# zju3dv/NeuralRecon-W

Hardware: NVIDIA H100
Metric: training rays/sec (higher is better)
Workload: dtype bf16 (3-product split forward, plain bf16 backward, fp32 accumulate)

## Files before the change

### neuralrecon-w_b200/csrc/epilogue_fast.cuh

```cuda
#pragma once
#include "epilogue_tc.cuh"

namespace nrw {

enum EpiKind {
  EK_GENERIC = 0,
  EK_FWD_SOFTPLUS,
  EK_FWD_RELU,
  EK_FWD_NONE,
  EK_GATE_FWD,
  EK_TANGENT,
  EK_REVERSE,
  EK_RELU_BWD,
  EK_FWD_HEAD,
  EK_COUNT
};

inline int pick_epi_kind(const Epi& e) {
  auto al16 = [](const void* p) { return (reinterpret_cast<uintptr_t>(p) & 15) == 0; };
  auto rows16 = [&](const void* p, int ld) { return !p || (al16(p) && (ld & 3) == 0); };
  if (e.head_w || e.head_partial)
    return (e.head_w && e.head_partial && e.bias && al16(e.bias) && al16(e.head_w) && e.act == ACT_SOFTPLUS100 && e.scale == 1.0f && e.n_planes == 0 &&
            !e.atomic && !e.aux_u.p && !e.rowvec && !e.aux_relu && !e.out_pre && !e.out2 && !e.out_f32 &&
            !e.colsum && !e.aux_add && e.n_store >= (1 << 29)) ? EK_FWD_HEAD : -1;
  if (e.atomic || e.n_planes > 3) return EK_GENERIC;
  if (e.n_planes > 0 && (!al16(e.out_pl.p) || (e.out_pl.ld & 3) || (e.out_pl.pstride & 7))) return EK_GENERIC;
  if (e.aux_u.p && (!al16(e.aux_u.p) || (e.aux_u.ld & 3) || (e.aux_u.pstride & 7))) return EK_GENERIC;
  if (!rows16(e.out_pre.p, e.out_pre.ld) || !rows16(e.out2.p, e.out2.ld) || !rows16(e.aux_add.p, e.aux_add.ld) ||
      !rows16(e.aux_q.p, e.aux_q_bcast ? 0 : e.aux_q.ld) || !rows16(e.out_f32, e.ld_f32) || !rows16(e.aux_relu, e.ld_relu) ||
      !al16(e.bias) || !al16(e.colvec))
    return EK_GENERIC;
  const bool gate = e.aux_u.p != nullptr;
  if (gate && e.out_pre && !e.out2 && !e.aux_add && !e.colsum && !e.bias && !e.rowvec && !e.aux_relu && e.n_planes > 0 && !e.out_f32)
    return EK_GATE_FWD;
  if (gate && e.out2 && e.aux_q && !e.out_pre && !e.bias && !e.rowvec && !e.aux_add && !e.colsum && !e.aux_relu &&
      ((e.n_planes > 0) != (e.out_f32 != nullptr)))
    return EK_TANGENT;
  if (gate && e.aux_add && !e.out2 && !e.out_pre && !e.bias && !e.aux_relu && e.n_planes > 0 && !e.out_f32) return EK_REVERSE;
  if (!gate && e.aux_relu && !e.out_pre && !e.out2 && !e.aux_add && !e.bias && e.n_planes > 0 && !e.out_f32 && e.act == ACT_NONE)
    return EK_RELU_BWD;
  if (!gate && e.bias && !e.rowvec && !e.aux_relu && !e.aux_add && !e.out_pre && !e.out2 && !e.out_f32 && !e.colsum && e.n_planes > 0) {
    if (e.act == ACT_SOFTPLUS100) return EK_FWD_SOFTPLUS;
    if (e.act == ACT_RELU) return EK_FWD_RELU;
    if (e.act == ACT_NONE) return EK_FWD_NONE;
  }
  return EK_GENERIC;
}

#define NRW_GATE_K (-144.269504088896341f)

template <int EK>
__device__ __forceinline__ void epi_fast16(const Epi& e, float* stg, const float (&v)[16], int m0w, int nc, int M, int N, int lane,
                                           float* cs_tile, float* hacc) {
  if constexpr (EK == EK_GENERIC) {
    epi_chunk16(e, stg, v, m0w, nc, M, N, lane, cs_tile);
  } else if constexpr (EK == EK_FWD_HEAD) {
    const int col = nc + (lane & 3) * 4;
    const float4 b = ldg4(e.bias + col), hw = ldg4(e.head_w + col);
    float x[16];
    line_transpose(stg, v, lane, x);
#pragma unroll
    for (int it = 0; it < 4; ++it) {
      float p = softplus100(x[4 * it] + b.x) * hw.x;
      p = fmaf(softplus100(x[4 * it + 1] + b.y), hw.y, p);
      p = fmaf(softplus100(x[4 * it + 2] + b.z), hw.z, p);
      p = fmaf(softplus100(x[4 * it + 3] + b.w), hw.w, p);
      p += __shfl_xor_sync(0xFFFFFFFFu, p, 1);
      p += __shfl_xor_sync(0xFFFFFFFFu, p, 2);
      hacc[it] += p;
    }
  } else {
    if (M - m0w < 32 || N - nc < 16 || e.n_store - nc < 16) {
      epi_chunk16(e, stg, v, m0w, nc, M, N, lane, cs_tile);
      return;
    }
    const int col = nc + (lane & 3) * 4;
    const long long row = (long long)m0w + (lane >> 2);
    float u[16];
    float s[16];
    float4 b;
    if constexpr (EK == EK_GATE_FWD || EK == EK_TANGENT || EK == EK_REVERSE) {
      tile_load_bf16(e.aux_u.p + row * e.aux_u.ld + col, e.aux_u.ld, u);
      if constexpr (EK == EK_GATE_FWD) {
        if (e.aux_u_planes > 1) tile_load_bf16(e.aux_u.plane(1) + row * e.aux_u.ld + col, e.aux_u.ld, s);
      }
    }
    if constexpr (EK == EK_FWD_SOFTPLUS || EK == EK_FWD_RELU || EK == EK_FWD_NONE) b = ldg4(e.bias + col);
    if constexpr (EK == EK_TANGENT) {
      if (e.aux_q_bcast) {
        const float4 qb = ldg4(e.aux_q.f32() + col);
#pragma unroll
        for (int it = 0; it < 4; ++it) { s[4 * it] = qb.x; s[4 * it + 1] = qb.y; s[4 * it + 2] = qb.z; s[4 * it + 3] = qb.w; }
      } else {
        tile_load(e.aux_q, row, col, s);
      }
    }
    if constexpr (EK == EK_REVERSE) tile_load(e.aux_add, row, col, s);
    if constexpr (EK == EK_RELU_BWD) tile_load_bf16(e.aux_relu + row * e.ld_relu + col, e.ld_relu, u);
    float x[16], w[16];
    line_transpose(stg, v, lane, x);

    if constexpr (EK == EK_FWD_SOFTPLUS || EK == EK_FWD_RELU || EK == EK_FWD_NONE) {
      const float bb[4] = {b.x, b.y, b.z, b.w};
#pragma unroll
      for (int i = 0; i < 16; ++i) {
        const float t = x[i] + bb[i & 3];
        if constexpr (EK == EK_FWD_SOFTPLUS) w[i] = softplus100(t) * e.scale;
        else if constexpr (EK == EK_FWD_RELU) w[i] = fmaxf(t, 0.0f) * e.scale;
        else w[i] = t * e.scale;
      }
    }
    if constexpr (EK == EK_REVERSE || EK == EK_RELU_BWD) {
      if (e.rowvec) {
        const float4 c = ldg4(e.colvec + col);
        const float cc[4] = {c.x, c.y, c.z, c.w};
#pragma unroll
        for (int it = 0; it < 4; ++it) {
          const float rv = __ldg(e.rowvec + row + it * 8);
#pragma unroll
          for (int k = 0; k < 4; ++k) x[4 * it + k] = fmaf(rv, cc[k], x[4 * it + k]);
        }
      }
    }
    if constexpr (EK == EK_GATE_FWD) tile_store(e.out_pre, row, col, x);
    if constexpr (EK == EK_GATE_FWD || EK == EK_TANGENT || EK == EK_REVERSE) {
      if constexpr (EK == EK_GATE_FWD) {
        if (e.aux_u_planes > 1) {
#pragma unroll
          for (int i = 0; i < 16; ++i) u[i] += s[i];
        }
      }
      for (int pl = EK == EK_GATE_FWD ? 2 : 1; pl < e.aux_u_planes; ++pl) {
        float t[16];
        tile_load_bf16(e.aux_u.plane(pl) + row * e.aux_u.ld + col, e.aux_u.ld, t);
#pragma unroll
        for (int i = 0; i < 16; ++i) u[i] += t[i];
      }
      const float kk = NRW_GATE_K * e.aux_u_scale, sc = e.scale;
      if constexpr (EK == EK_TANGENT) {
        const float sc100 = 100.0f * sc;
#pragma unroll
        for (int i = 0; i < 16; ++i) {
          const float ee = mufu_ex2(u[i] * kk);
          const float s1 = 1.0f - ee;
          const float xs = x[i] * s1;
          w[i] = xs * sc;
          s[i] = (xs * s[i]) * (ee * sc100);
        }
        tile_store(e.out2, row, col, s);
      } else if constexpr (EK == EK_REVERSE) {
#pragma unroll
        for (int i = 0; i < 16; ++i) {
          const float ee = mufu_ex2(u[i] * kk);
          w[i] = fmaf(x[i], fmaf(-sc, ee, sc), s[i]);
        }
      } else {
#pragma unroll
        for (int i = 0; i < 16; ++i) {
          const float ee = mufu_ex2(u[i] * kk);
          w[i] = x[i] * fmaf(-sc, ee, sc);
        }
      }
    }
    if constexpr (EK == EK_RELU_BWD) {
#pragma unroll
      for (int i = 0; i < 16; ++i) w[i] = u[i] > 0.0f ? x[i] * e.scale : 0.0f;
    }
    if constexpr (EK == EK_REVERSE || EK == EK_RELU_BWD) {
      if (cs_tile) line_colsum_add(w, lane, cs_tile);
    }
    if constexpr (EK == EK_TANGENT) {
      if (e.out_f32) tile_store_f32(e.out_f32 + row * e.ld_f32 + col, e.ld_f32, w);
    }
    for (int pl = 0; pl < e.n_planes; ++pl) {
      uint32_t pk[8];
      if (pl + 1 < e.n_planes) split_plane<16>(w, pk);
      else pack_bf16(w, pk);
      tile_store_bf16(e.out_pl.plane(pl) + row * e.out_pl.ld + col, e.out_pl.ld, pk);
    }
  }
}

}
```

### neuralrecon-w_b200/csrc/epilogue_tc.cuh

```cuda
#pragma once
#include "epilogue.cuh"

namespace nrw {

struct LineLayout {
  int sl;
  int r0;
  int rows_valid;
  bool full;
};

__device__ __forceinline__ bool aligned16(const void* p) { return (reinterpret_cast<uintptr_t>(p) & 15) == 0; }
__device__ __forceinline__ bool aligned8(const void* p) { return (reinterpret_cast<uintptr_t>(p) & 7) == 0; }

__device__ __forceinline__ void line_transpose(float* stg, const float (&v)[16], int lane, float (&x)[16]) {
  const int sl = lane & 3, r0 = lane >> 2;
#pragma unroll
  for (int s = 0; s < 4; ++s)
    *reinterpret_cast<float4*>(stg + lane * 16 + ((s ^ ((lane >> 1) & 3)) << 2)) = make_float4(v[4 * s], v[4 * s + 1], v[4 * s + 2], v[4 * s + 3]);
  __syncwarp();
#pragma unroll
  for (int it = 0; it < 4; ++it) {
    const int rr = it * 8 + r0;
    const float4 t = *reinterpret_cast<const float4*>(stg + rr * 16 + ((sl ^ ((rr >> 1) & 3)) << 2));
    x[4 * it] = t.x; x[4 * it + 1] = t.y; x[4 * it + 2] = t.z; x[4 * it + 3] = t.w;
  }
  __syncwarp();
}

__device__ __forceinline__ float4 ldg4(const float* p) {
  float4 v;
  asm volatile("ld.global.nc.L2::256B.v4.f32 {%0, %1, %2, %3}, [%4];" : "=f"(v.x), "=f"(v.y), "=f"(v.z), "=f"(v.w) : "l"(p));
  return v;
}
__device__ __forceinline__ uint2 ldg2u(const bf16* p) {
  uint2 v;
  asm volatile("ld.global.nc.L2::256B.v2.u32 {%0, %1}, [%2];" : "=r"(v.x), "=r"(v.y) : "l"(p));
  return v;
}

__device__ __forceinline__ void tile_load_f32(const float* p, long long ld, float (&o)[16]) {
#pragma unroll
  for (int it = 0; it < 4; ++it) {
    const float4 t = ldg4(p + it * 8 * ld);
    o[4 * it] = t.x; o[4 * it + 1] = t.y; o[4 * it + 2] = t.z; o[4 * it + 3] = t.w;
  }
}
__device__ __forceinline__ void tile_load_bf16(const bf16* p, long long ld, float (&o)[16]) {
#pragma unroll
  for (int it = 0; it < 4; ++it) {
    const uint2 t = ldg2u(p + it * 8 * ld);
    o[4 * it] = __uint_as_float(t.x << 16); o[4 * it + 1] = __uint_as_float(t.x & 0xFFFF0000u);
    o[4 * it + 2] = __uint_as_float(t.y << 16); o[4 * it + 3] = __uint_as_float(t.y & 0xFFFF0000u);
  }
}
__device__ __forceinline__ void tile_store_f32(float* p, long long ld, const float (&o)[16]) {
#pragma unroll
  for (int it = 0; it < 4; ++it)
    *reinterpret_cast<float4*>(p + it * 8 * ld) = make_float4(o[4 * it], o[4 * it + 1], o[4 * it + 2], o[4 * it + 3]);
}
__device__ __forceinline__ void tile_store_bf16(bf16* p, long long ld, const uint32_t (&pk)[8]) {
#pragma unroll
  for (int it = 0; it < 4; ++it) *reinterpret_cast<uint2*>(p + it * 8 * ld) = make_uint2(pk[2 * it], pk[2 * it + 1]);
}
__device__ __forceinline__ void pack_bf16(const float (&w)[16], uint32_t (&pk)[8]) {
#pragma unroll
  for (int t = 0; t < 8; ++t) {
    const __nv_bfloat162 h = __floats2bfloat162_rn(w[2 * t], w[2 * t + 1]);
    pk[t] = *reinterpret_cast<const uint32_t*>(&h);
  }
}
__device__ __forceinline__ void tile_load(const SideStream& s, long long row, int col, float (&o)[16]) {
  if (s.is_bf16()) tile_load_bf16(s.h() + row * s.ld + col, s.ld, o);
  else tile_load_f32(s.f32() + row * s.ld + col, s.ld, o);
}
__device__ __forceinline__ void tile_store(const SideStream& s, long long row, int col, const float (&o)[16]) {
  if (s.is_bf16()) {
    uint32_t pk[8];
    pack_bf16(o, pk);
    tile_store_bf16(s.h() + row * s.ld + col, s.ld, pk);
  } else {
    tile_store_f32(s.f32() + row * s.ld + col, s.ld, o);
  }
}

__device__ __forceinline__ bool line_fast(const LineLayout& L, const void* p, long long ld, int ncols) {
  return L.full && ncols >= 16 && aligned16(p) && (ld & 3) == 0;
}
__device__ __forceinline__ void line_load_f32(const LineLayout& L, const float* __restrict__ src, long long ld, int ncols,
                                              float (&o)[16]) {
  if (line_fast(L, src, ld, ncols)) {
    tile_load_f32(src + L.r0 * ld + L.sl * 4, ld, o);
    return;
  }
#pragma unroll
  for (int it = 0; it < 4; ++it) {
    const int rr = it * 8 + L.r0;
#pragma unroll
    for (int k = 0; k < 4; ++k) {
      const int c = L.sl * 4 + k;
      o[4 * it + k] = (rr < L.rows_valid && c < ncols) ? src[(long long)rr * ld + c] : 0.0f;
    }
  }
}
__device__ __forceinline__ void line_store_f32(const LineLayout& L, float* __restrict__ dst, long long ld, int ncols,
                                               const float (&o)[16], bool atomic) {
  if (!atomic && line_fast(L, dst, ld, ncols)) {
    tile_store_f32(dst + L.r0 * ld + L.sl * 4, ld, o);
    return;
  }
#pragma unroll
  for (int it = 0; it < 4; ++it) {
    const int rr = it * 8 + L.r0;
#pragma unroll
    for (int k = 0; k < 4; ++k) {
      const int c = L.sl * 4 + k;
      if (rr < L.rows_valid && c < ncols) {
        if (atomic) atomicAdd(dst + (long long)rr * ld + c, o[4 * it + k]);
        else dst[(long long)rr * ld + c] = o[4 * it + k];
      }
    }
  }
}
__device__ __forceinline__ void line_store_bf16(const LineLayout& L, bf16* __restrict__ dst, long long ld, int ncols,
                                                const uint32_t (&pk)[8]) {
  if (L.full && ncols >= 16 && aligned8(dst) && (ld & 3) == 0) {
    tile_store_bf16(dst + L.r0 * ld + L.sl * 4, ld, pk);
    return;
  }
#pragma unroll
  for (int it = 0; it < 4; ++it) {
// ... 9 lines not shown
__device__ __forceinline__ void line_load_planes(const LineLayout& L, const Planes& P, int n_planes, long long m0w, int nc, int ncols,
                                                 float scale, float (&o)[16]) {
#pragma unroll
  for (int i = 0; i < 16; ++i) o[i] = 0.0f;
  for (int pl = 0; pl < n_planes; ++pl) {
    const bf16* src = P.plane(pl) + m0w * P.ld + nc;
    if (L.full && ncols >= 16 && aligned8(src) && (P.ld & 3) == 0) {
      float t[16];
      tile_load_bf16(src + L.r0 * P.ld + L.sl * 4, P.ld, t);
#pragma unroll
      for (int i = 0; i < 16; ++i) o[i] += t[i];
    } else {
#pragma unroll
      for (int it = 0; it < 4; ++it) {
        const int rr = it * 8 + L.r0;
#pragma unroll
        for (int k = 0; k < 4; ++k) {
          const int c = L.sl * 4 + k;
          if (rr < L.rows_valid && c < ncols) o[4 * it + k] += __bfloat162float(src[(long long)rr * P.ld + c]);
        }
      }
    }
  }
  if (scale != 1.0f) {
#pragma unroll
    for (int i = 0; i < 16; ++i) o[i] *= scale;
  }
}
__device__ __forceinline__ void line_load_cols(const LineLayout& L, const float* __restrict__ vec, int ncols, float (&b)[4]) {
  const float* p = vec + L.sl * 4;
  if (ncols >= 16 && aligned16(vec)) {
    const float4 t = __ldg(reinterpret_cast<const float4*>(p));
    b[0] = t.x; b[1] = t.y; b[2] = t.z; b[3] = t.w;
  } else {
#pragma unroll
    for (int k = 0; k < 4; ++k) b[k] = (L.sl * 4 + k < ncols) ? p[k] : 0.0f;
  }
}
__device__ __forceinline__ void line_load(const LineLayout& L, const SideStream& s, long long m0w, int nc, int ncols, float (&o)[16]) {
  if (s.is_bf16()) line_load_planes(L, Planes{s.h(), 0, s.ld}, 1, m0w, nc, ncols, 1.0f, o);
  else line_load_f32(L, s.f32() + m0w * s.ld + nc, s.ld, ncols, o);
}
__device__ __forceinline__ void line_store(const LineLayout& L, const SideStream& s, long long m0w, int nc, int ncols,
                                           const float (&o)[16]) {
  if (s.is_bf16()) {
    uint32_t pk[8];
    pack_bf16(o, pk);
    line_store_bf16(L, s.h() + m0w * s.ld + nc, s.ld, ncols, pk);
  } else {
    line_store_f32(L, s.f32() + m0w * s.ld + nc, s.ld, ncols, o, false);
  }
}

__device__ __forceinline__ void line_colsum_add(const float (&w)[16], int lane, float* cs_tile) {
  float c0 = (w[0] + w[4]) + (w[8] + w[12]), c1 = (w[1] + w[5]) + (w[9] + w[13]);
  float c2 = (w[2] + w[6]) + (w[10] + w[14]), c3 = (w[3] + w[7]) + (w[11] + w[15]);
  const bool hi16 = (lane & 16) != 0, hi8 = (lane & 8) != 0;
  const float s0 = hi16 ? c0 : c2, s1 = hi16 ? c1 : c3;
  float k0 = hi16 ? c2 : c0, k1 = hi16 ? c3 : c1;
  k0 += __shfl_xor_sync(0xFFFFFFFFu, s0, 16);
  k1 += __shfl_xor_sync(0xFFFFFFFFu, s1, 16);
  const float s = hi8 ? k0 : k1;
  float k = hi8 ? k1 : k0;
  k += __shfl_xor_sync(0xFFFFFFFFu, s, 8);
  k += __shfl_xor_sync(0xFFFFFFFFu, k, 4);
  if ((lane & 4) == 0) atomicAdd(cs_tile + (lane & 3) * 4 + (hi16 ? 2 : 0) + (hi8 ? 1 : 0), k);
}

__device__ __forceinline__ void epi_chunk16(const Epi& e, float* stg, const float (&v)[16], int m0w, int nc, int M, int N, int lane,
                                            float* cs_tile) {
  LineLayout L;
  L.rows_valid = min(32, M - m0w);
  if (L.rows_valid <= 0) return;
  const int n_all = min(N - nc, 16);
  const int n_st = min(e.n_store - nc, n_all);
  L.sl = lane & 3;
  L.r0 = lane >> 2;
  L.full = L.rows_valid == 32;
  float x[16];
  line_transpose(stg, v, lane, x);
  if (e.bias) {
    float b[4];
    line_load_cols(L, e.bias + nc, n_all, b);
#pragma unroll
    for (int i = 0; i < 16; ++i) x[i] += b[i & 3];
  }
  if (e.rowvec) {
    float cv[4];
    line_load_cols(L, e.colvec + nc, n_all, cv);
#pragma unroll
    for (int it = 0; it < 4; ++it) {
      const float rv = e.rowvec[min(m0w + it * 8 + L.r0, M - 1)];
#pragma unroll
      for (int k = 0; k < 4; ++k) x[4 * it + k] = fmaf(rv, cv[k], x[4 * it + k]);
    }
  }
  if (e.out_pre) line_store(L, e.out_pre, m0w, nc, n_all, x);
  if (n_st <= 0) return;
  if (e.atomic) {
    if (e.scale != 1.0f) {
#pragma unroll
      for (int i = 0; i < 16; ++i) x[i] *= e.scale;
    }
    line_store_f32(L, e.out_f32 + (long long)m0w * e.ld_f32 + nc, e.ld_f32, n_st, x, true);
    return;
  }
  float w[16];
  if (e.aux_u.p) {
    float a[16];
    line_load_planes(L, e.aux_u, e.aux_u_planes, m0w, nc, n_st, e.aux_u_scale, a);
    if (e.out2) {
      float q[16];
      if (e.aux_q_bcast) {
        float qb[4];
        line_load_cols(L, e.aux_q.f32() + nc, n_st, qb);
#pragma unroll
        for (int i = 0; i < 16; ++i) q[i] = qb[i & 3];
      } else {
        line_load(L, e.aux_q, m0w, nc, n_st, q);
      }
#pragma unroll
      for (int i = 0; i < 16; ++i) {
        float s1, s2;
        softplus100_d12_from_u(a[i], s1, s2);
        w[i] = x[i] * s1 * e.scale;
        q[i] = e.scale * x[i] * q[i] * s2;
      }
      line_store(L, e.out2, m0w, nc, n_st, q);
    } else {
#pragma unroll
      for (int i = 0; i < 16; ++i) {
        float s1, s2;
        softplus100_d12_from_u(a[i], s1, s2);
        w[i] = x[i] * s1 * e.scale;
      }
    }
  } else {
    switch (e.act) {
      case ACT_SOFTPLUS100:
#pragma unroll
        for (int i = 0; i < 16; ++i) w[i] = softplus100(x[i]) * e.scale;
        break;
      case ACT_RELU:
#pragma unroll
        for (int i = 0; i < 16; ++i) w[i] = fmaxf(x[i], 0.0f) * e.scale;
        break;
      case ACT_SIGMOID:
#pragma unroll
        for (int i = 0; i < 16; ++i) w[i] = sigmoidf_(x[i]) * e.scale;
        break;
      default:
#pragma unroll
        for (int i = 0; i < 16; ++i) w[i] = x[i] * e.scale;
    }
    if (e.aux_relu) {
      float f[16];
      line_load_planes(L, Planes{const_cast<bf16*>(e.aux_relu), 0, e.ld_relu}, 1, m0w, nc, n_st, 1.0f, f);
#pragma unroll
      for (int i = 0; i < 16; ++i)
        if (!(f[i] > 0.0f)) w[i] = 0.0f;
    }
  }
  if (e.aux_add) {
    float ad[16];
    line_load(L, e.aux_add, m0w, nc, n_st, ad);
#pragma unroll
    for (int i = 0; i < 16; ++i) w[i] += ad[i];
  }
  if (cs_tile) {
#pragma unroll
    for (int i = 0; i < 16; ++i)
      if ((i >> 2) * 8 + L.r0 >= L.rows_valid || L.sl * 4 + (i & 3) >= n_st) w[i] = 0.0f;
    line_colsum_add(w, lane, cs_tile);
  }
  if (e.out_f32) line_store_f32(L, e.out_f32 + (long long)m0w * e.ld_f32 + nc, e.ld_f32, n_st, w, false);
  for (int pl = 0; pl < e.n_planes; ++pl) {
    uint32_t pk[8];
    split_plane<16>(w, pk);
    line_store_bf16(L, e.out_pl.plane(pl) + (long long)m0w * e.out_pl.ld + nc, e.out_pl.ld, n_st, pk);
  }
}

__device__ __forceinline__ void colsum_flush(float* cs, float* __restrict__ colsum, int n0, int n_cols, int tid, int n_threads,
                                             int bar_id) {
  asm volatile("bar.sync %0, %1;" ::"r"(bar_id), "r"(n_threads) : "memory");
  for (int i = tid; i < n_cols; i += n_threads) {
    const float s = cs[i];
    if (i < n_cols && s != 0.0f) atomicAdd(colsum + n0 + i, s);
    cs[i] = 0.0f;
  }
  asm volatile("bar.sync %0, %1;" ::"r"(bar_id), "r"(n_threads) : "memory");
}

}
```

### neuralrecon-w_b200/csrc/gemm_tc.cu

```cuda
#include <stdlib.h>

#include <mutex>
#include <unordered_map>
#include <vector>
#include <algorithm>
#include <stdio.h>

#include "gemm.h"
#include "epilogue_fast.cuh"

namespace nrw {

static constexpr int BM = 128;
static constexpr int BK = 64;
static constexpr int RING_BYTES = 192 * 1024;
static constexpr int MAX_STAGES = 8;
static constexpr int N_CONSUMER_WARPS = 8;
static constexpr int N_THREADS = 32 * N_CONSUMER_WARPS + 128;
static constexpr int PRODUCER_REGS = 40, CONSUMER_REGS = 232;
static constexpr int EPI_LD = 36;
static constexpr int EPI_WG_BYTES = 64 * EPI_LD * 4;
static constexpr int CS_BYTES = 1024;
static constexpr int BAR_TURN = 4;
static_assert(PRODUCER_REGS * 128 + CONSUMER_REGS * 32 * N_CONSUMER_WARPS <= 65536, "register file");
// ... 238 lines not shown
      if ((j & 1) != wg) {
        for (int kb = kb0; kb < kb1; ++kb)
          if (++s == stages) { s = 0; ph ^= 1; }
        continue;
      }
      if (use_cs && n0 != cs_n0) {
        if (cs_n0 >= 0) colsum_flush(cs_wg, p.epi.colsum, cs_n0, min(min(p.N, p.epi.n_store) - cs_n0, BN), ctid, 128, 2 + wg);
        cs_n0 = n0;
      }
      float acc[2][BN / 2];
#pragma unroll
      for (int h = 0; h < 2; ++h)
#pragma unroll
        for (int i = 0; i < BN / 2; ++i) acc[h][i] = 0.0f;
      if (j > 0) {
        NRW_PROF_T0(prof);
        named_bar_sync(BAR_TURN + wg, 256);
        NRW_PROF_ADD(prof, 3 + po);
      }
      int prev_s = -1;
      for (int kb = kb0; kb < kb1; ++kb) {
        {
          NRW_PROF_T0(prof);
          mbar_wait(bar_full + 8 * s, ph);
          NRW_PROF_ADD(prof, 1 + po);
        }
        const uint32_t sa = smem0 + s * stage_bytes;
        const uint32_t sb = smem0 + s * stage_bytes + P * A_TILE;
        wgmma_fence();
        for (int pr = 0; pr < n_prod; ++pr) {
          const int q = 4 * (n_prod - 1 - pr);
          const uint32_t pa = (0x021010u >> q) & 0xFu, pb = (0x201100u >> q) & 0xFu;
          const uint64_t da = desc_hi | (uint64_t)(((sa + pa * A_TILE) & 0x3FFFFu) >> 4);
          const uint64_t db = desc_hi | (uint64_t)(((sb + pb * B_TILE) & 0x3FFFFu) >> 4);
#pragma unroll
          for (int k = 0; k < BK / 16; ++k)
#pragma unroll
            for (int h = 0; h < 2; ++h)
              wgmma_bf16<BN, MN_MAJOR, MN_MAJOR>(acc[h], da + ((h * WG_A + k * KSTEP) >> 4), db + ((k * KSTEP) >> 4), 1u);
        }
        wgmma_commit();
        acc_fence(acc[0]);
        acc_fence(acc[1]);
        if (prev_s >= 0) {
          wgmma_wait<1>();
          acc_fence(acc[0]);
          acc_fence(acc[1]);
          if (lane == 0) mbar_arrive(bar_empty + 8 * prev_s);
        }
        prev_s = s;
        if (++s == stages) { s = 0; ph ^= 1; }
      }
      if (item + gridDim.x < n_items) named_bar_arrive(BAR_TURN + (wg ^ 1), 256);
      wgmma_wait<0>();
      acc_fence(acc[0]);
      acc_fence(acc[1]);
      if (prev_s >= 0 && lane == 0) mbar_arrive(bar_empty + 8 * prev_s);
      if (kb1 <= kb0) continue;
      NRW_PROF_T0(prof);
      if (prof) atomicAdd(&p.prof[blockIdx.x * 16 + 6 + po], 1ull);
      const int r0 = 16 * wi + (lane >> 2), c0 = 2 * (lane & 3);
      const int qq = wi & 1, cc = wi >> 1;
      const int n_cp = (min(BN, p.N - n0) + 31) / 32;
#pragma unroll
      for (int h = 0; h < 2; ++h) {
        const int m0w = m0 + 64 * h + 32 * qq;
        float hacc[4] = {0.0f, 0.0f, 0.0f, 0.0f};
#pragma unroll
        for (int cp = 0; cp < BN / 32; ++cp) {
          if (cp >= n_cp) break;
#pragma unroll
          for (int jj = 0; jj < 4; ++jj) {
            const int jf = 4 * cp + jj;
            *reinterpret_cast<float2*>(stage_tile + r0 * EPI_LD + 8 * jj + c0) = make_float2(acc[h][4 * jf], acc[h][4 * jf + 1]);
            *reinterpret_cast<float2*>(stage_tile + (r0 + 8) * EPI_LD + 8 * jj + c0) = make_float2(acc[h][4 * jf + 2], acc[h][4 * jf + 3]);
          }
          named_bar_sync(2 + wg, 128);
          float v[16];
          const float* src = stage_tile + (32 * qq + lane) * EPI_LD + 16 * cc;
#pragma unroll
          for (int i = 0; i < 4; ++i) {
            const float4 t4 = *reinterpret_cast<const float4*>(src + 4 * i);
            v[4 * i] = t4.x; v[4 * i + 1] = t4.y; v[4 * i + 2] = t4.z; v[4 * i + 3] = t4.w;
          }
          named_bar_sync(2 + wg, 128);
          const int nc = n0 + 32 * cp + 16 * cc;
          if (nc < p.N && m0w < p.M)
            epi_fast16<EK>(p.epi, stg, v, m0w, nc, p.M, p.N, lane, use_cs ? cs_wg + 32 * cp + 16 * cc : nullptr, hacc);
          named_bar_sync(2 + wg, 128);
        }
        if (EK == EK_FWD_HEAD && (lane & 3) == 0) {
          const int slot = (n0 / BN) * 2 + cc;
#pragma unroll
          for (int it = 0; it < 4; ++it) {
            const int row = m0w + it * 8 + (lane >> 2);
            if (row < p.M) p.epi.head_partial[(long long)row * 8 + slot] = hacc[it];
          }
        }
      }
      NRW_PROF_ADD(prof, 4 + po);
    }
    if (use_cs && cs_n0 >= 0) colsum_flush(cs_wg, p.epi.colsum, cs_n0, min(min(p.N, p.epi.n_store) - cs_n0, BN), ctid, 128, 2 + wg);
  }
  __syncthreads();
  if (p.prof && threadIdx.x == 0) atomicAdd(&p.prof[blockIdx.x * 16 + 5], (unsigned long long)(clock64() - t_kernel0));
}

typedef CUresult (*EncodeTiledFn)(CUtensorMap*, CUtensorMapDataType, cuuint32_t, void*, const cuuint64_t*,
                                  const cuuint64_t*, const cuuint32_t*, const cuuint32_t*,
                                  CUtensorMapInterleave, CUtensorMapSwizzle, CUtensorMapL2promotion,
                                  CUtensorMapFloatOOBfill);

static EncodeTiledFn get_encode() {
  static EncodeTiledFn fn = nullptr;
  static std::once_flag once;
  std::call_once(once, [] {
// ... 136 lines not shown
  const Epi& e = g.epi;
  const int q_bytes = e.aux_q_bcast ? 0 : e.aux_q.elem_bytes();
  L.epi = (e.out_pre ? 1u : 0u) | (e.out_f32 ? 2u : 0u) | (e.out2 ? 4u : 0u) | (e.n_planes ? 8u : 0u) | (e.aux_u.p ? 16u : 0u) |
          (q_bytes ? 32u : 0u) | (e.aux_add ? 64u : 0u) | (e.aux_relu ? 128u : 0u) | (e.atomic ? 256u : 0u) | (e.colsum ? 512u : 0u);
  const double mn = (double)g.M * (double)std::min(g.N, e.n_store);
  L.bytes = 2.0 * g.n_planes * ((double)g.M * g.K + (double)g.N * g.K) + (double)e.out_pre.elem_bytes() * g.M * g.N +
            mn * (4.0 * (e.out_f32 ? 1 : 0) + e.out2.elem_bytes() + q_bytes + e.aux_add.elem_bytes() + 2.0 * e.n_planes +
                  (e.aux_relu ? 2.0 : 0.0) + (e.aux_u.p ? 2.0 * e.aux_u_planes : 0.0));
  NRW_CUDA_OK(cudaEventRecord(L.e0, stream));
  const int rc = gemm_tc_impl(g, stream);
  NRW_CUDA_OK(cudaEventRecord(L.e1, stream));
  g_timed.push_back(L);
  return rc;
}
static int gemm_tc_impl(const GemmDesc& g, cudaStream_t stream) {
  NRW_CHECK(g.M > 0 && g.N > 0 && g.K > 0, NRW_ERR_ARG, "gemm_tc: empty problem %d %d %d", g.M, g.N, g.K);
  NRW_CHECK(g.n_planes >= 1 && g.n_planes <= 3, NRW_ERR_ARG, "gemm_tc: n_planes=%d", g.n_planes);
  NRW_CHECK(g.k_slices == 1 || g.epi.atomic, NRW_ERR_ARG, "gemm_tc: split-K needs an atomic epilogue");
  static int n_sm_dev[MAX_DEV] = {0};
  const int dev = current_device();
  if (!n_sm_dev[dev]) NRW_CUDA_OK(cudaDeviceGetAttribute(&n_sm_dev[dev], cudaDevAttrMultiProcessorCount, dev));
  const int n_sm = n_sm_dev[dev];
  const int BN = g.N <= 64 ? 64 : 128;
  TcParams p;
  memset(&p, 0, sizeof(p));
  p.M = g.M; p.N = g.N; p.K = g.K; p.n_planes = g.n_planes; p.k_slices = g.k_slices;
  p.m_tiles = cdiv(g.M, BM); p.n_tiles = cdiv(g.N, BN);
  p.epi = g.epi;
  p.prof = g_prof_ptr;
  for (int pl = 0; pl < g.n_planes; ++pl) {
    if (!g.mn_major) {
      NRW_CHECK(g.K % BK == 0, NRW_ERR_ARG, "gemm_tc: K=%d must be a multiple of %d (pad the operand)", g.K, BK);
      NRW_TRY(make_map(&p.tmA[pl], g.A.plane(pl), g.K, g.M, g.A.ld, BK, BM));
      NRW_TRY(make_map(&p.tmB[pl], g.B.plane(pl), g.K, g.N, g.B.ld, BK, BN));
    } else {
      NRW_TRY(make_map(&p.tmA[pl], g.A.plane(pl), g.M, g.K, g.A.ld, 64, BK));
      NRW_TRY(make_map(&p.tmB[pl], g.B.plane(pl), g.N, g.K, g.B.ld, 64, BK));
    }
  }
  const int ek = g.mn_major ? EK_GENERIC : pick_epi_kind(g.epi);
  NRW_CHECK(ek >= 0 && (ek != EK_FWD_HEAD || g.N == 512), NRW_ERR_ARG,
            "gemm_tc: the fused SDF-head epilogue needs N = 512, bias + softplus and no other output");
  if (g.mn_major) return BN == 64 ? launch<64, 1, EK_GENERIC>(p, n_sm, dev, stream) : launch<128, 1, EK_GENERIC>(p, n_sm, dev, stream);
  if (BN == 64) return launch<64, 0, EK_GENERIC>(p, n_sm, dev, stream);
  switch (ek) {
    case EK_FWD_SOFTPLUS: return launch<128, 0, EK_FWD_SOFTPLUS>(p, n_sm, dev, stream);
    case EK_FWD_RELU: return launch<128, 0, EK_FWD_RELU>(p, n_sm, dev, stream);
    case EK_FWD_NONE: return launch<128, 0, EK_FWD_NONE>(p, n_sm, dev, stream);
    case EK_FWD_HEAD: return launch<128, 0, EK_FWD_HEAD>(p, n_sm, dev, stream);
    case EK_GATE_FWD: return launch<128, 0, EK_GATE_FWD>(p, n_sm, dev, stream);
    case EK_TANGENT: return launch<128, 0, EK_TANGENT>(p, n_sm, dev, stream);
    case EK_REVERSE: return launch<128, 0, EK_REVERSE>(p, n_sm, dev, stream);
    case EK_RELU_BWD: return launch<128, 0, EK_RELU_BWD>(p, n_sm, dev, stream);
    default: return launch<128, 0, EK_GENERIC>(p, n_sm, dev, stream);
  }
}


static constexpr int FZ_ROWS = 64;
static constexpr int FZ_APLANE = FZ_ROWS * 512 * 2;
static constexpr int FZ_A = 2 * FZ_APLANE;
static constexpr int FZ_WG = 4;
static constexpr int FZ_WSTAGE = 64 * BK * 2;
static constexpr int FZ_NST = 3;
static constexpr int FZ_BAR = FZ_A + FZ_WG * FZ_NST * FZ_WSTAGE;
static constexpr int FZ_SMEM = 1024 + FZ_BAR + 256;
static constexpr int FZ_THREADS = 128 * FZ_WG;
static constexpr int FZ_POS_PER_TILE = 4 * (1 + 7 * 8);
static_assert(FZ_SMEM <= 232448, "dynamic shared memory limit of sm_90");

struct SdfFusedParams {
  CUtensorMap tmW[8][2];
  const float* bias[8];
  const float* head_w;
  const float* head_b;
  const float* pts;
  float* sdf;
  int M, n_tiles;
};

__device__ __forceinline__ float pe6_feature(const float (&x)[3], int f) {
  if (f < 3) return x[f];
  const int k = (f - 3) / 6, wi = (f - 3) % 6, c = wi % 3;
  float sn, cs;
  sincosf(x[c] * (float)(1 << k), &sn, &cs);
  return wi < 3 ? sn : cs;
}

__global__ void __launch_bounds__(FZ_THREADS, 1) sdf_fused_kernel(const __grid_constant__ SdfFusedParams p) {
  extern __shared__ uint8_t smem_raw[];
  uint8_t* smem = smem_raw + ((1024u - (smem_u32(smem_raw) & 1023u)) & 1023u);
  uint64_t* bars = reinterpret_cast<uint64_t*>(smem + FZ_BAR);
  const uint32_t w_full = smem_u32(bars);
  const int warp = threadIdx.x >> 5, lane = threadIdx.x & 31;
  const uint32_t smem0 = smem_u32(smem);
  const int g = warp >> 2, wi = warp & 3, et = threadIdx.x;
  const bool loader = wi == 0 && lane == 0;

  if (et == 0) {
    for (int l = 0; l < 8; ++l) { tma_prefetch_desc(&p.tmW[l][0]); tma_prefetch_desc(&p.tmW[l][1]); }
    for (int i = 0; i < FZ_WG * FZ_NST; ++i) mbar_init(w_full + 8 * i, 1);
    asm volatile("fence.mbarrier_init.release.cluster;" ::: "memory");
  }
  __syncthreads();
  pdl_wait();
  pdl_launch_dependents();
// ... 211 lines not shown
```

Baseline: 34650.

## Run GEMM epilogue directly on wgmma fragments with prefetched side inputs

For the forward bias/activation kernels and ReLU backward, full tiles now run the epilogue straight from the wgmma accumulator registers, using a lane shuffle exchange instead of staging through shared memory with named barriers. Side inputs (bias, relu mask) are prefetched as raw words before the wgmma wait and then software-pipelined one slice ahead. The tile helpers are templated on size, and a new LINEAR_BWD fast kind covers plain scaled backward outputs that previously took the generic path. The cost is more register pressure from the prefetch buffers plus extra shuffles, and the colsum atomics move from one shared tile to per-column addresses.

Result: faster. 36090 (median of 6 runs) (+4.2%).

```diff
diff --git a/neuralrecon-w_b200/csrc/epilogue_fast.cuh b/neuralrecon-w_b200/csrc/epilogue_fast.cuh
--- a/neuralrecon-w_b200/csrc/epilogue_fast.cuh
+++ b/neuralrecon-w_b200/csrc/epilogue_fast.cuh
@@ -12,6 +12,7 @@
   EK_TANGENT,
   EK_REVERSE,
   EK_RELU_BWD,
+  EK_LINEAR_BWD,
   EK_FWD_HEAD,
   EK_COUNT
 };
@@ -37,8 +38,8 @@
       ((e.n_planes > 0) != (e.out_f32 != nullptr)))
     return EK_TANGENT;
   if (gate && e.aux_add && !e.out2 && !e.out_pre && !e.bias && !e.aux_relu && e.n_planes > 0 && !e.out_f32) return EK_REVERSE;
-  if (!gate && e.aux_relu && !e.out_pre && !e.out2 && !e.aux_add && !e.bias && e.n_planes > 0 && !e.out_f32 && e.act == ACT_NONE)
-    return EK_RELU_BWD;
+  if (!gate && !e.out_pre && !e.out2 && !e.aux_add && !e.bias && e.n_planes > 0 && !e.out_f32 && e.act == ACT_NONE)
+    return e.aux_relu ? EK_RELU_BWD : EK_LINEAR_BWD;
   if (!gate && e.bias && !e.rowvec && !e.aux_relu && !e.aux_add && !e.out_pre && !e.out2 && !e.out_f32 && !e.colsum && e.n_planes > 0) {
     if (e.act == ACT_SOFTPLUS100) return EK_FWD_SOFTPLUS;
     if (e.act == ACT_RELU) return EK_FWD_RELU;
@@ -48,6 +49,152 @@
 }
 
 #define NRW_GATE_K (-144.269504088896341f)
+
+__host__ __device__ constexpr bool frag_kind(int ek) {
+  return ek == EK_FWD_SOFTPLUS || ek == EK_FWD_RELU || ek == EK_FWD_NONE || ek == EK_RELU_BWD;
+}
+
+template <int N>
+struct FastIn {
+  uint32_t u[N / 2];
+  uint32_t u2[N / 2];
+  uint32_t s[N];
+  float4 b;
+};
+
+template <int EK, int N>
+__device__ __forceinline__ void fast_load(const Epi& e, long long row, int col, FastIn<N>& in) {
+  if constexpr (EK == EK_GATE_FWD || EK == EK_TANGENT || EK == EK_REVERSE) {
+    tile_load_bf16_raw(e.aux_u.p + row * e.aux_u.ld + col, e.aux_u.ld, in.u);
+    if constexpr (EK == EK_GATE_FWD) {
+      if (e.aux_u_planes > 1) tile_load_bf16_raw(e.aux_u.plane(1) + row * e.aux_u.ld + col, e.aux_u.ld, in.u2);
+    }
+  }
+  if constexpr (EK == EK_FWD_SOFTPLUS || EK == EK_FWD_RELU || EK == EK_FWD_NONE) in.b = ldg4(e.bias + col);
+  if constexpr (EK == EK_TANGENT) {
+    if (e.aux_q_bcast) in.b = ldg4(e.aux_q.f32() + col);
+    else tile_load_raw(e.aux_q, row, col, in.s);
+  }
+  if constexpr (EK == EK_REVERSE) tile_load_raw(e.aux_add, row, col, in.s);
+  if constexpr (EK == EK_RELU_BWD) tile_load_bf16_raw(e.aux_relu + row * e.ld_relu + col, e.ld_relu, in.u);
+}
+
+template <int EK, int N>
+__device__ __forceinline__ void fast_tile(const Epi& e, float (&x)[N], const FastIn<N>& in, long long row, int col, float* cs_lane,
+                                          int lane) {
+  float w[N];
+  if constexpr (EK == EK_FWD_SOFTPLUS || EK == EK_FWD_RELU || EK == EK_FWD_NONE) {
+    const float bb[4] = {in.b.x, in.b.y, in.b.z, in.b.w};
+#pragma unroll
+    for (int i = 0; i < N; ++i) {
+      const float t = x[i] + bb[i & 3];
+      if constexpr (EK == EK_FWD_SOFTPLUS) w[i] = softplus100(t) * e.scale;
+      else if constexpr (EK == EK_FWD_RELU) w[i] = fmaxf(t, 0.0f) * e.scale;
+      else w[i] = t * e.scale;
+    }
+  }
+  if constexpr (EK == EK_REVERSE || EK == EK_RELU_BWD || EK == EK_LINEAR_BWD) {
+    if (e.rowvec) {
+      const float4 c = ldg4(e.colvec + col);
+      const float cc[4] = {c.x, c.y, c.z, c.w};
+#pragma unroll
+      for (int it = 0; it < N / 4; ++it) {
+        const float rv = __ldg(e.rowvec + row + it * 8);
+#pragma unroll
+        for (int k = 0; k < 4; ++k) x[4 * it + k] = fmaf(rv, cc[k], x[4 * it + k]);
+      }
+    }
+  }
+  if constexpr (EK == EK_GATE_FWD) tile_store(e.out_pre, row, col, x);
+  if constexpr (EK == EK_GATE_FWD || EK == EK_TANGENT || EK == EK_REVERSE) {
+    float u[N], s[N];
+    unpack_bf16(in.u, u);
+    if constexpr (EK == EK_GATE_FWD) {
+      if (e.aux_u_planes > 1) {
+        unpack_bf16(in.u2, s);
+#pragma unroll
+        for (int i = 0; i < N; ++i) u[i] += s[i];
+      }
+    }
+    if constexpr (EK == EK_TANGENT) {
+      if (e.aux_q_bcast) {
+        const float qb[4] = {in.b.x, in.b.y, in.b.z, in.b.w};
+#pragma unroll
+        for (int i = 0; i < N; ++i) s[i] = qb[i & 3];
+      } else {
+        unpack_side(e.aux_q, in.s, s);
+      }
+    }
+    if constexpr (EK == EK_REVERSE) unpack_side(e.aux_add, in.s, s);
+    for (int pl = EK == EK_GATE_FWD ? 2 : 1; pl < e.aux_u_planes; ++pl) {
+      float t[N];
+      tile_load_bf16(e.aux_u.plane(pl) + row * e.aux_u.ld + col, e.aux_u.ld, t);
+#pragma unroll
+      for (int i = 0; i < N; ++i) u[i] += t[i];
+    }
+    const float kk = NRW_GATE_K * e.aux_u_scale, sc = e.scale;
+    if constexpr (EK == EK_TANGENT) {
+      const float sc100 = 100.0f * sc;
+#pragma unroll
+      for (int i = 0; i < N; ++i) {
+        const float ee = mufu_ex2(u[i] * kk);
+        const float s1 = 1.0f - ee;
+        const float xs = x[i] * s1;
+        w[i] = xs * sc;
+        s[i] = (xs * s[i]) * (ee * sc100);
+      }
+      tile_store(e.out2, row, col, s);
+    } else if constexpr (EK == EK_REVERSE) {
+#pragma unroll
+      for (int i = 0; i < N; ++i) {
+        const float ee = mufu_ex2(u[i] * kk);
+        w[i] = fmaf(x[i], fmaf(-sc, ee, sc), s[i]);
+      }
+    } else {
+#pragma unroll
+      for (int i = 0; i < N; ++i) {
+        const float ee = mufu_ex2(u[i] * kk);
+        w[i] = x[i] * fmaf(-sc, ee, sc);
+      }
+    }
+  }
+  if constexpr (EK == EK_RELU_BWD) {
+    float f[N];
+    unpack_bf16(in.u, f);
+#pragma unroll
+    for (int i = 0; i < N; ++i) w[i] = f[i] > 0.0f ? x[i] * e.scale : 0.0f;
+  }
+  if constexpr (EK == EK_LINEAR_BWD) {
+#pragma unroll
+    for (int i = 0; i < N; ++i) w[i] = x[i] * e.scale;
+  }
+  if constexpr (EK == EK_REVERSE || EK == EK_RELU_BWD || EK == EK_LINEAR_BWD) {
+    if (cs_lane) colsum_add(w, lane, cs_lane);
+  }
+  if constexpr (EK == EK_TANGENT) {
+    if (e.out_f32) tile_store_f32(e.out_f32 + row * e.ld_f32 + col, e.ld_f32, w);
+  }
+  for (int pl = 0; pl < e.n_planes; ++pl) {
+    uint32_t pk[N / 2];
+    if (pl + 1 < e.n_planes) split_plane<N>(w, pk);
+    else pack_bf16(w, pk);
+    tile_store_bf16(e.out_pl.plane(pl) + row * e.out_pl.ld + col, e.out_pl.ld, pk);
+  }
+}
+
+__device__ __forceinline__ int frag_col(int lane) { return 4 * ((lane >> 1) & 1) + 8 * (lane & 1); }
+template <int NA>
+__device__ __forceinline__ void frag_exchange(const float (&a)[NA], int jp, int lane, float (&x)[8]) {
+  const bool odd = (lane & 1) != 0;
+#pragma unroll
+  for (int r = 0; r < 2; ++r) {
+    const int j = 2 * jp;
+    const float a0 = a[4 * j + 2 * r], a1 = a[4 * j + 2 * r + 1], b0 = a[4 * j + 4 + 2 * r], b1 = a[4 * j + 5 + 2 * r];
+    const float t0 = __shfl_xor_sync(0xFFFFFFFFu, odd ? a0 : b0, 1), t1 = __shfl_xor_sync(0xFFFFFFFFu, odd ? a1 : b1, 1);
+    x[4 * r] = odd ? t0 : a0; x[4 * r + 1] = odd ? t1 : a1;
+    x[4 * r + 2] = odd ? b0 : t0; x[4 * r + 3] = odd ? b1 : t1;
+  }
+}
 
 template <int EK>
 __device__ __forceinline__ void epi_fast16(const Epi& e, float* stg, const float (&v)[16], int m0w, int nc, int M, int N, int lane,
@@ -76,109 +223,12 @@
     }
     const int col = nc + (lane & 3) * 4;
     const long long row = (long long)m0w + (lane >> 2);
-    float u[16];
-    float s[16];
-    float4 b;
-    if constexpr (EK == EK_GATE_FWD || EK == EK_TANGENT || EK == EK_REVERSE) {
-      tile_load_bf16(e.aux_u.p + row * e.aux_u.ld + col, e.aux_u.ld, u);
-      if constexpr (EK == EK_GATE_FWD) {
-        if (e.aux_u_planes > 1) tile_load_bf16(e.aux_u.plane(1) + row * e.aux_u.ld + col, e.aux_u.ld, s);
-      }
-    }
-    if constexpr (EK == EK_FWD_SOFTPLUS || EK == EK_FWD_RELU || EK == EK_FWD_NONE) b = ldg4(e.bias + col);
-    if constexpr (EK == EK_TANGENT) {
-      if (e.aux_q_bcast) {
-        const float4 qb = ldg4(e.aux_q.f32() + col);
-#pragma unroll
-        for (int it = 0; it < 4; ++it) { s[4 * it] = qb.x; s[4 * it + 1] = qb.y; s[4 * it + 2] = qb.z; s[4 * it + 3] = qb.w; }
-      } else {
-        tile_load(e.aux_q, row, col, s);
-      }
-    }
-    if constexpr (EK == EK_REVERSE) tile_load(e.aux_add, row, col, s);
-    if constexpr (EK == EK_RELU_BWD) tile_load_bf16(e.aux_relu + row * e.ld_relu + col, e.ld_relu, u);
-    float x[16], w[16];
+    FastIn<16> in;
+    fast_load<EK>(e, row, col, in);
+    float x[16];
     line_transpose(stg, v, lane, x);
-
-    if constexpr (EK == EK_FWD_SOFTPLUS || EK == EK_FWD_RELU || EK == EK_FWD_NONE) {
-      const float bb[4] = {b.x, b.y, b.z, b.w};
-#pragma unroll
-      for (int i = 0; i < 16; ++i) {
-        const float t = x[i] + bb[i & 3];
-        if constexpr (EK == EK_FWD_SOFTPLUS) w[i] = softplus100(t) * e.scale;
-        else if constexpr (EK == EK_FWD_RELU) w[i] = fmaxf(t, 0.0f) * e.scale;
-        else w[i] = t * e.scale;
-      }
-    }
-    if constexpr (EK == EK_REVERSE || EK == EK_RELU_BWD) {
-      if (e.rowvec) {
-        const float4 c = ldg4(e.colvec + col);
-        const float cc[4] = {c.x, c.y, c.z, c.w};
-#pragma unroll
-        for (int it = 0; it < 4; ++it) {
-          const float rv = __ldg(e.rowvec + row + it * 8);
-#pragma unroll
-          for (int k = 0; k < 4; ++k) x[4 * it + k] = fmaf(rv, cc[k], x[4 * it + k]);
-        }
-      }
-    }
-    if constexpr (EK == EK_GATE_FWD) tile_store(e.out_pre, row, col, x);
-    if constexpr (EK == EK_GATE_FWD || EK == EK_TANGENT || EK == EK_REVERSE) {
-      if constexpr (EK == EK_GATE_FWD) {
-        if (e.aux_u_planes > 1) {
-#pragma unroll
-          for (int i = 0; i < 16; ++i) u[i] += s[i];
-        }
-      }
-      for (int pl = EK == EK_GATE_FWD ? 2 : 1; pl < e.aux_u_planes; ++pl) {
-        float t[16];
-        tile_load_bf16(e.aux_u.plane(pl) + row * e.aux_u.ld + col, e.aux_u.ld, t);
-#pragma unroll
-        for (int i = 0; i < 16; ++i) u[i] += t[i];
-      }
-      const float kk = NRW_GATE_K * e.aux_u_scale, sc = e.scale;
-      if constexpr (EK == EK_TANGENT) {
-        const float sc100 = 100.0f * sc;
-#pragma unroll
-        for (int i = 0; i < 16; ++i) {
-          const float ee = mufu_ex2(u[i] * kk);
-          const float s1 = 1.0f - ee;
-          const float xs = x[i] * s1;
-          w[i] = xs * sc;
-          s[i] = (xs * s[i]) * (ee * sc100);
-        }
-        tile_store(e.out2, row, col, s);
-      } else if constexpr (EK == EK_REVERSE) {
-#pragma unroll
-        for (int i = 0; i < 16; ++i) {
-          const float ee = mufu_ex2(u[i] * kk);
-          w[i] = fmaf(x[i], fmaf(-sc, ee, sc), s[i]);
-        }
-      } else {
-#pragma unroll
-        for (int i = 0; i < 16; ++i) {
-          const float ee = mufu_ex2(u[i] * kk);
-          w[i] = x[i] * fmaf(-sc, ee, sc);
-        }
-      }
-    }
-    if constexpr (EK == EK_RELU_BWD) {
-#pragma unroll
-      for (int i = 0; i < 16; ++i) w[i] = u[i] > 0.0f ? x[i] * e.scale : 0.0f;
-    }
-    if constexpr (EK == EK_REVERSE || EK == EK_RELU_BWD) {
-      if (cs_tile) line_colsum_add(w, lane, cs_tile);
-    }
-    if constexpr (EK == EK_TANGENT) {
-      if (e.out_f32) tile_store_f32(e.out_f32 + row * e.ld_f32 + col, e.ld_f32, w);
-    }
-    for (int pl = 0; pl < e.n_planes; ++pl) {
-      uint32_t pk[8];
-      if (pl + 1 < e.n_planes) split_plane<16>(w, pk);
-      else pack_bf16(w, pk);
-      tile_store_bf16(e.out_pl.plane(pl) + row * e.out_pl.ld + col, e.out_pl.ld, pk);
-    }
-  }
-}
-
-}
+    fast_tile<EK>(e, x, in, row, col, cs_tile ? cs_tile + (lane & 3) * 4 : nullptr, lane);
+  }
+}
+
+}
diff --git a/neuralrecon-w_b200/csrc/epilogue_tc.cuh b/neuralrecon-w_b200/csrc/epilogue_tc.cuh
--- a/neuralrecon-w_b200/csrc/epilogue_tc.cuh
+++ b/neuralrecon-w_b200/csrc/epilogue_tc.cuh
@@ -39,44 +39,88 @@
   return v;
 }
 
-__device__ __forceinline__ void tile_load_f32(const float* p, long long ld, float (&o)[16]) {
-#pragma unroll
-  for (int it = 0; it < 4; ++it) {
+template <int N>
+__device__ __forceinline__ void tile_load_f32(const float* p, long long ld, float (&o)[N]) {
+#pragma unroll
+  for (int it = 0; it < N / 4; ++it) {
     const float4 t = ldg4(p + it * 8 * ld);
     o[4 * it] = t.x; o[4 * it + 1] = t.y; o[4 * it + 2] = t.z; o[4 * it + 3] = t.w;
   }
 }
-__device__ __forceinline__ void tile_load_bf16(const bf16* p, long long ld, float (&o)[16]) {
-#pragma unroll
-  for (int it = 0; it < 4; ++it) {
+template <int N>
+__device__ __forceinline__ void tile_load_bf16_raw(const bf16* p, long long ld, uint32_t (&r)[N]) {
+#pragma unroll
+  for (int it = 0; it < N / 2; ++it) {
     const uint2 t = ldg2u(p + it * 8 * ld);
-    o[4 * it] = __uint_as_float(t.x << 16); o[4 * it + 1] = __uint_as_float(t.x & 0xFFFF0000u);
-    o[4 * it + 2] = __uint_as_float(t.y << 16); o[4 * it + 3] = __uint_as_float(t.y & 0xFFFF0000u);
-  }
-}
-__device__ __forceinline__ void tile_store_f32(float* p, long long ld, const float (&o)[16]) {
-#pragma unroll
-  for (int it = 0; it < 4; ++it)
+    r[2 * it] = t.x; r[2 * it + 1] = t.y;
+  }
+}
+template <int N>
+__device__ __forceinline__ void unpack_bf16(const uint32_t (&r)[N], float (&o)[2 * N]) {
+#pragma unroll
+  for (int t = 0; t < N; ++t) { o[2 * t] = __uint_as_float(r[t] << 16); o[2 * t + 1] = __uint_as_float(r[t] & 0xFFFF0000u); }
+}
+template <int N>
+__device__ __forceinline__ void tile_load_bf16(const bf16* p, long long ld, float (&o)[N]) {
+  uint32_t r[N / 2];
+  tile_load_bf16_raw(p, ld, r);
+  unpack_bf16(r, o);
+}
+template <int N>
+__device__ __forceinline__ void tile_store_f32(float* p, long long ld, const float (&o)[N]) {
+#pragma unroll
+  for (int it = 0; it < N / 4; ++it)
     *reinterpret_cast<float4*>(p + it * 8 * ld) = make_float4(o[4 * it], o[4 * it + 1], o[4 * it + 2], o[4 * it + 3]);
 }
-__device__ __forceinline__ void tile_store_bf16(bf16* p, long long ld, const uint32_t (&pk)[8]) {
-#pragma unroll
-  for (int it = 0; it < 4; ++it) *reinterpret_cast<uint2*>(p + it * 8 * ld) = make_uint2(pk[2 * it], pk[2 * it + 1]);
-}
-__device__ __forceinline__ void pack_bf16(const float (&w)[16], uint32_t (&pk)[8]) {
-#pragma unroll
-  for (int t = 0; t < 8; ++t) {
+template <int N>
+__device__ __forceinline__ void tile_store_bf16(bf16* p, long long ld, const uint32_t (&pk)[N]) {
+#pragma unroll
+  for (int it = 0; it < N / 2; ++it) *reinterpret_cast<uint2*>(p + it * 8 * ld) = make_uint2(pk[2 * it], pk[2 * it + 1]);
+}
+template <int N>
+__device__ __forceinline__ void pack_bf16(const float (&w)[N], uint32_t (&pk)[N / 2]) {
+#pragma unroll
+  for (int t = 0; t < N / 2; ++t) {
     const __nv_bfloat162 h = __floats2bfloat162_rn(w[2 * t], w[2 * t + 1]);
     pk[t] = *reinterpret_cast<const uint32_t*>(&h);
   }
 }
-__device__ __forceinline__ void tile_load(const SideStream& s, long long row, int col, float (&o)[16]) {
-  if (s.is_bf16()) tile_load_bf16(s.h() + row * s.ld + col, s.ld, o);
-  else tile_load_f32(s.f32() + row * s.ld + col, s.ld, o);
-}
-__device__ __forceinline__ void tile_store(const SideStream& s, long long row, int col, const float (&o)[16]) {
+template <int N>
+__device__ __forceinline__ void tile_load_raw(const SideStream& s, long long row, int col, uint32_t (&r)[N]) {
   if (s.is_bf16()) {
-    uint32_t pk[8];
+    uint32_t t[N / 2];
+    tile_load_bf16_raw(s.h() + row * s.ld + col, s.ld, t);
+#pragma unroll
+    for (int i = 0; i < N / 2; ++i) r[i] = t[i];
+  } else {
+    float o[N];
+    tile_load_f32(s.f32() + row * s.ld + col, s.ld, o);
+#pragma unroll
+    for (int i = 0; i < N; ++i) r[i] = __float_as_uint(o[i]);
+  }
+}
+template <int N>
+__device__ __forceinline__ void unpack_side(const SideStream& s, const uint32_t (&r)[N], float (&o)[N]) {
+  if (s.is_bf16()) {
+    uint32_t t[N / 2];
+#pragma unroll
+    for (int i = 0; i < N / 2; ++i) t[i] = r[i];
+    unpack_bf16(t, o);
+  } else {
+#pragma unroll
+    for (int i = 0; i < N; ++i) o[i] = __uint_as_float(r[i]);
+  }
+}
+template <int N>
+__device__ __forceinline__ void tile_load(const SideStream& s, long long row, int col, float (&o)[N]) {
+  uint32_t r[N];
+  tile_load_raw(s, row, col, r);
+  unpack_side(s, r, o);
+}
+template <int N>
+__device__ __forceinline__ void tile_store(const SideStream& s, long long row, int col, const float (&o)[N]) {
+  if (s.is_bf16()) {
+    uint32_t pk[N / 2];
     pack_bf16(o, pk);
     tile_store_bf16(s.h() + row * s.ld + col, s.ld, pk);
   } else {
@@ -192,9 +236,15 @@
   }
 }
 
-__device__ __forceinline__ void line_colsum_add(const float (&w)[16], int lane, float* cs_tile) {
-  float c0 = (w[0] + w[4]) + (w[8] + w[12]), c1 = (w[1] + w[5]) + (w[9] + w[13]);
-  float c2 = (w[2] + w[6]) + (w[10] + w[14]), c3 = (w[3] + w[7]) + (w[11] + w[15]);
+template <int N>
+__device__ __forceinline__ void colsum_add(const float (&w)[N], int lane, float* cs_lane) {
+  float c0, c1, c2, c3;
+  if constexpr (N == 16) {
+    c0 = (w[0] + w[4]) + (w[8] + w[12]); c1 = (w[1] + w[5]) + (w[9] + w[13]);
+    c2 = (w[2] + w[6]) + (w[10] + w[14]); c3 = (w[3] + w[7]) + (w[11] + w[15]);
+  } else {
+    c0 = w[0] + w[4]; c1 = w[1] + w[5]; c2 = w[2] + w[6]; c3 = w[3] + w[7];
+  }
   const bool hi16 = (lane & 16) != 0, hi8 = (lane & 8) != 0;
   const float s0 = hi16 ? c0 : c2, s1 = hi16 ? c1 : c3;
   float k0 = hi16 ? c2 : c0, k1 = hi16 ? c3 : c1;
@@ -204,7 +254,7 @@
   float k = hi8 ? k1 : k0;
   k += __shfl_xor_sync(0xFFFFFFFFu, s, 8);
   k += __shfl_xor_sync(0xFFFFFFFFu, k, 4);
-  if ((lane & 4) == 0) atomicAdd(cs_tile + (lane & 3) * 4 + (hi16 ? 2 : 0) + (hi8 ? 1 : 0), k);
+  if ((lane & 4) == 0) atomicAdd(cs_lane + (hi16 ? 2 : 0) + (hi8 ? 1 : 0), k);
 }
 
 __device__ __forceinline__ void epi_chunk16(const Epi& e, float* stg, const float (&v)[16], int m0w, int nc, int M, int N, int lane,
@@ -311,7 +361,7 @@
 #pragma unroll
     for (int i = 0; i < 16; ++i)
       if ((i >> 2) * 8 + L.r0 >= L.rows_valid || L.sl * 4 + (i & 3) >= n_st) w[i] = 0.0f;
-    line_colsum_add(w, lane, cs_tile);
+    colsum_add(w, lane, cs_tile + L.sl * 4);
   }
   if (e.out_f32) line_store_f32(L, e.out_f32 + (long long)m0w * e.ld_f32 + nc, e.ld_f32, n_st, w, false);
   for (int pl = 0; pl < e.n_planes; ++pl) {
diff --git a/neuralrecon-w_b200/csrc/gemm_tc.cu b/neuralrecon-w_b200/csrc/gemm_tc.cu
--- a/neuralrecon-w_b200/csrc/gemm_tc.cu
+++ b/neuralrecon-w_b200/csrc/gemm_tc.cu
@@ -314,6 +314,14 @@
         if (++s == stages) { s = 0; ph ^= 1; }
       }
       if (item + gridDim.x < n_items) named_bar_arrive(BAR_TURN + (wg ^ 1), 256);
+      const int r0 = 16 * wi + (lane >> 2), c0 = 2 * (lane & 3);
+      constexpr int NJP = BN / 16;
+      bool frag_epi = false;
+      FastIn<8> pf;
+      if constexpr (frag_kind(EK)) {
+        frag_epi = m0 + BM <= p.M && n0 + BN <= min(p.N, p.epi.n_store);
+        if (frag_epi) fast_load<EK>(p.epi, m0 + r0, n0 + frag_col(lane), pf);
+      }
       wgmma_wait<0>();
       acc_fence(acc[0]);
       acc_fence(acc[1]);
@@ -321,9 +329,24 @@
       if (kb1 <= kb0) continue;
       NRW_PROF_T0(prof);
       if (prof) atomicAdd(&p.prof[blockIdx.x * 16 + 6 + po], 1ull);
-      const int r0 = 16 * wi + (lane >> 2), c0 = 2 * (lane & 3);
+      if constexpr (frag_kind(EK)) {
+        if (frag_epi) {
+#pragma unroll
+          for (int sl = 0; sl < 2 * NJP; ++sl) {
+            const int h = sl / NJP, jp = sl % NJP;
+            FastIn<8> nx;
+            if (sl + 1 < 2 * NJP)
+              fast_load<EK>(p.epi, m0 + 64 * ((sl + 1) / NJP) + r0, n0 + 16 * ((sl + 1) % NJP) + frag_col(lane), nx);
+            float x[8];
+            frag_exchange(acc[h], jp, lane, x);
+            const int col = 16 * jp + frag_col(lane);
+            fast_tile<EK>(p.epi, x, pf, m0 + 64 * h + r0, n0 + col, use_cs ? cs_wg + col : nullptr, lane);
+            if (sl + 1 < 2 * NJP) pf = nx;
+          }
+        }
+      }
       const int qq = wi & 1, cc = wi >> 1;
-      const int n_cp = (min(BN, p.N - n0) + 31) / 32;
+      const int n_cp = frag_epi ? 0 : (min(BN, p.N - n0) + 31) / 32;
 #pragma unroll
       for (int h = 0; h < 2; ++h) {
         const int m0w = m0 + 64 * h + 32 * qq;
@@ -566,6 +589,7 @@
     case EK_TANGENT: return launch<128, 0, EK_TANGENT>(p, n_sm, dev, stream);
     case EK_REVERSE: return launch<128, 0, EK_REVERSE>(p, n_sm, dev, stream);
     case EK_RELU_BWD: return launch<128, 0, EK_RELU_BWD>(p, n_sm, dev, stream);
+    case EK_LINEAR_BWD: return launch<128, 0, EK_LINEAR_BWD>(p, n_sm, dev, stream);
     default: return launch<128, 0, EK_GENERIC>(p, n_sm, dev, stream);
   }
 }
```
